# zhujinchong/3DGS-native

Measured on AMD Instinct MI355X. Metric: Mpixels/s forward+backward at 800x800, 1M Gaussians, higher is better.
Workload: dtype f32

## Files before the change

### 3dgs-native_amd/csrc/api.hip

```cpp
#include <stdio.h>
#include <stdlib.h>
#include <string.h>

#include <algorithm>
#include <atomic>
#include <mutex>
#include <vector>

#include "gsr_antialias.h"
#include "gsr_aux_grads.h"
#include "gsr_camera_grads.h"
#include "gsr_capacity.h"
#include "gsr_debug_layout.h"
#include "gsr_densify_stats.h"
#include "gsr_internal.h"

namespace {

#define HIP_TRY(expr)                                                                                                         \
    do {                                                                                                                      \
        hipError_t e_ = (expr);                                                                                               \
        if (e_ != hipSuccess) {                                                                                               \
            fprintf(stderr, "libgsr_hip: %s failed at %s:%d: %s\n", #expr, __FILE__, __LINE__, hipGetErrorString(e_));       \
            return GSR_E_HIP;                                                                                                 \
        }                                                                                                                     \
    } while (0)

struct Carver {
    char *p;
    size_t off = 0;
    explicit Carver(void *base) : p((char *)base) {}
    template <class T> T *take(size_t count)
    {
        T *r = (T *)(p ? p + off : nullptr);
        off += gsr_align(count * sizeof(T));
        return r;
    }
};

BinWs carve_bin(void *base, int64_t D)
{
    Carver c(base);
    BinWs w;
    w.hist = c.take<int32_t>(256 * ((size_t)gsr_radix_blocks(D) + 1));
    w.acc[0] = c.take<int32_t>(gsr_radix_acc_ints(D));
    w.acc[1] = c.take<int32_t>(gsr_radix_acc_ints(D));
    w.edge = c.take<int32_t>(3 * 256 * ((size_t)gsr_radix_blocks(D) + 1));
    w.tile_a = c.take<uint64_t>((size_t)D);
    w.tile_b = c.take<uint64_t>((size_t)D);
    w.bytes = c.off + 256;
    return w;
}

struct BwdWs {
    BlendRec *rec;
    GradRec *acc;
    size_t bytes;
};
BwdWs carve_bwd(void *base, int64_t N)
{
    Carver c(base);
    BwdWs w;
    w.rec = c.take<BlendRec>((size_t)N);
    w.acc = c.take<GradRec>((size_t)N);
    w.bytes = c.off + 256;
    return w;
}

int check_scene_cam(const GsrScene *sc, const GsrCamera *cam)
{
// ... 347 lines not shown
    HIP_TRY(hipMemsetAsync(image->inv_depth, 0, P * sizeof(float), s));
    HIP_TRY(hipMemsetAsync(image->final_T, 0, P * sizeof(float), s));
    HIP_TRY(hipMemsetAsync(image->n_contrib, 0, P * sizeof(int32_t), s));
    if (binning->backward_ws && N > 0) HIP_TRY(hipMemsetAsync(carve_bwd(binning->backward_ws, N).acc, 0, sizeof(GradRec) * (size_t)N, s));
    return GSR_OK;
}

int enqueue_render(const GsrScene *scene, const CamK &cam, const GsrGeom *geom, const GsrBinning *binning, const GsrImage *image,
                   const GeomWs &gw, const BinWs &bw, const int32_t *d_count, int64_t shape_D, hipStream_t s, int st)
{
    const int64_t N = scene->N, D = binning->D;
    const int tiles = cam.grid_x * cam.grid_y;
    if (!d_count) shape_D = D;
    mark(st, 4, s);
    const TilePlan plan = gsr_tile_plan(N, tiles);
    int32_t *order = binning->block_masks ? binning->block_order : nullptr;
    const bool file_order = order && tiles <= GSR_BO_MAX_TILES && gsr_bwd_block_px(N, shape_D, tiles) == 32;
    const bool use_fwd_order = fwd_order_wanted(tiles);
    HIP_TRY(gsr_launch_depth_block_offsets(gw, N, binning->ranges, 2 * tiles, bw.acc[0], (int)gsr_radix_acc_ints(D), order, order ? GSR_BO_HEADER : 0,
                                           file_order ? 1 : 0, s));
    mark(st, 5, s);
    HIP_TRY(gsr_launch_expand_blocks(plan, gw, bw, N, cam.grid_x, D, d_count, s));
    mark(st, 6, s);
    HIP_TRY(gsr_launch_tile_partition(plan, bw, binning->point_list, binning->ranges, D, d_count, s));
    mark(st, 7, s);
    mark(st, 8, s);
    void *clear = binning->backward_ws ? carve_bwd(binning->backward_ws, N).acc : nullptr;
    const size_t clear_bytes = clear ? sizeof(GradRec) * (size_t)N : 0;
    HIP_TRY(gsr_launch_blend_forward(cam, binning->ranges, binning->point_list, geom->blend_records ? (const BlendRec *)geom->blend_records : gw.rec, *image, binning->block_masks, file_order ? order : nullptr,
                                     clear, clear_bytes, s, use_fwd_order ? gw.fwd_order : nullptr, tiles <= GSR_FO_MAX_TILES ? gw.fwd_cost : nullptr,
                                     d_count, D));
    mark(st, 9, s);
    return GSR_OK;
}

}

extern "C" {

int gsr_forward_render(const GsrScene *scene, const GsrCamera *camera, const GsrGeom *geom, const GsrBinning *binning,
                       const GsrImage *image, void *geom_ws, size_t geom_ws_bytes, void *bin_ws, size_t bin_ws_bytes, void *stream)
{
    read_tuning();
    if (int rc = check_frame(scene, camera, binning, image)) return rc;
    const int64_t N = scene->N, D = binning->D;
    hipStream_t s = (hipStream_t)stream;
    const CamK cam = make_cam(camera);
// ... 314 lines not shown
```

### 3dgs-native_amd/csrc/gsr_internal.h

```cpp
#pragma once
#include <hip/hip_runtime.h>
#include <stdint.h>

#include "gsr.h"

#define GSR_WAVE 64

struct CamK {
    float view[16];
    float proj[16];
    float campos[3];
    float bg[3];
    float tan_fovx, tan_fovy;
    float focal_x, focal_y;
    int W, H, grid_x, grid_y;
};

struct __attribute__((aligned(16))) BlendRec {
    float f[16];
};

struct __attribute__((aligned(8))) TileRect {
    uint16_t x0, y0, x1, y1;
};
// ... 83 lines not shown
static inline int gsr_radix_sb(int nb)
{
    if (nb > GSR_RADIX_PREFIX_NB) return 32;
    int sb = 16;
    while ((int64_t)sb * sb < nb) ++sb;
    return sb;
}
static inline size_t gsr_radix_acc_ints(int64_t n)
{
    const int nb = (int)gsr_radix_blocks(n), sb = gsr_radix_sb(nb);
    return 256 * (size_t)(3 + nb / sb);
}
struct TilePlan {
    int tile_bits, id_bits;
    int item_bytes, id_shift;
    int npass;
    int bits[4];
    bool narrowing;
};
TilePlan gsr_tile_plan(int64_t N, int tiles);
struct BinWs {
    int32_t *hist;
    int32_t *acc[2];
    int32_t *edge;
    uint64_t *tile_a;
    uint64_t *tile_b;
    size_t bytes;
};
hipError_t gsr_launch_depth_block_offsets(const GeomWs &ws, int64_t n, int32_t *ranges, int ranges_n, int32_t *zero_acc, int zero_n, int32_t *zero_b,
                                          int zero_b_n, int bo_flag, hipStream_t s);
hipError_t gsr_launch_expand_blocks(const TilePlan &plan, const GeomWs &ws, const BinWs &bw, int64_t n, int grid_x, int64_t D, const int32_t *d_count,
                                    hipStream_t s);
hipError_t gsr_launch_tile_partition(const TilePlan &plan, const BinWs &bw, int32_t *point_list, int32_t *ranges, int64_t D, const int32_t *d_count,
                                     hipStream_t s);
#define GSR_BO_BANDS 8
#define GSR_BO_CLASSES 32
#define GSR_BO_SHARDS 16
#define GSR_BO_QUEUES (GSR_BO_BANDS * GSR_BO_CLASSES * GSR_BO_SHARDS)
#define GSR_BO_FLAG GSR_BO_QUEUES
#define GSR_BO_HEADER (GSR_BO_QUEUES + 4)
#define GSR_BO_MAX_TILES 4096
__host__ __device__ static inline int gsr_bo_tiles_per_band(int tiles) { return (tiles + GSR_BO_BANDS - 1) / GSR_BO_BANDS; }
__host__ __device__ static inline int gsr_bo_band(int tile, int tiles) { return tile / gsr_bo_tiles_per_band(tiles); }
static inline int gsr_bo_cap(int tiles) { return 8 * ((gsr_bo_tiles_per_band(tiles) + GSR_BO_SHARDS - 1) / GSR_BO_SHARDS); }
static inline size_t gsr_bo_ints(int tiles) { return GSR_BO_HEADER + (size_t)GSR_BO_QUEUES * (size_t)gsr_bo_cap(tiles); }
__host__ __device__ static inline int gsr_bo_class(int hits)
{
    if (hits < 8) return 0;
    const int lg = 31 - __builtin_clz((unsigned)hits);
    const int c = 1 + 4 * (lg - 3) + ((hits >> (lg - 2)) & 3);
    return c < GSR_BO_CLASSES ? c : GSR_BO_CLASSES - 1;
}
hipError_t gsr_launch_blend_forward(const CamK &cam, const int32_t *ranges, const int32_t *point_list,
                                    const BlendRec *rec, const GsrImage &img, uint8_t *block_masks ,
                                    int32_t *block_order ,
                                    void *clear, size_t clear_bytes , hipStream_t s,
                                    const int32_t *tile_order = nullptr , int32_t *tile_cost = nullptr ,
// ... 43 lines not shown
```

### 3dgs-native_amd/csrc/scan_sort.hip

```cpp
#include <algorithm>
#include <type_traits>
#include <utility>

#include "gsr_internal.h"

namespace {

__device__ __forceinline__ int wave_incl_scan(int v)
{
    asm("s_nop 1\n\tv_add_u32_dpp %0, %0, %0 row_shr:1 row_mask:0xf bank_mask:0xf\n\t"
        "s_nop 1\n\tv_add_u32_dpp %0, %0, %0 row_shr:2 row_mask:0xf bank_mask:0xf\n\t"
        "s_nop 1\n\tv_add_u32_dpp %0, %0, %0 row_shr:4 row_mask:0xf bank_mask:0xf\n\t"
        "s_nop 1\n\tv_add_u32_dpp %0, %0, %0 row_shr:8 row_mask:0xf bank_mask:0xf\n\t"
        "s_nop 1\n\tv_add_u32_dpp %0, %0, %0 row_bcast:15 row_mask:0xa bank_mask:0xf\n\t"
        "s_nop 1\n\tv_add_u32_dpp %0, %0, %0 row_bcast:31 row_mask:0xc bank_mask:0xf\n\t"
        "s_nop 1"
        : "+v"(v));
    return v;
}

__device__ __forceinline__ int block_incl_scan_256(int v, int *lds4 , int *total)
{
    const int lane = threadIdx.x & 63, w = threadIdx.x >> 6;
    int s = wave_incl_scan(v);
// ... 179 lines not shown
    int launched_first;
    int pack_ok;
};
__device__ __forceinline__ bool depth_items_packed(const DepthPass &dp, const DepthCtl &c) { return dp.pack_ok && c.npass >= 2 && c.npass <= 3; }
__device__ __forceinline__ unsigned long long depth_item_pack(uint32_t key, unsigned long long rect_raw, uint32_t id)
{
    const uint32_t r24 = (uint32_t)(rect_raw & 63ull) | ((uint32_t)((rect_raw >> 16) & 63ull) << 6) | ((uint32_t)((rect_raw >> 32) & 63ull) << 12) |
                         ((uint32_t)((rect_raw >> 48) & 63ull) << 18);
    return ((unsigned long long)((key >> 8) & 0xFFFFu) << 48) | ((unsigned long long)r24 << 24) | (unsigned long long)(id & 0xFFFFFFu);
}
__device__ __forceinline__ unsigned long long depth_item_rect(unsigned long long item)
{
    const uint32_t r24 = (uint32_t)(item >> 24) & 0xFFFFFFu;
    return (unsigned long long)(r24 & 63u) | ((unsigned long long)((r24 >> 6) & 63u) << 16) | ((unsigned long long)((r24 >> 12) & 63u) << 32) |
           ((unsigned long long)((r24 >> 18) & 63u) << 48);
}
template <bool DEPTH, int BITS, typename ItemT>
__device__ __forceinline__ int radix_digit(ItemT item, int shift, uint32_t kmin, uint32_t krange)
{
    if constexpr (DEPTH) return (int)((min((uint32_t)(item >> 32) - kmin, krange) >> shift) & 255u);
    else return (int)((item >> shift) & ((1 << BITS) - 1));
}

template <int RADIX_ITEMS, int BITS, typename ItemT, bool DEPTH>
__device__ __forceinline__ void radix_hist_block(const ItemT *__restrict__ in, int32_t *__restrict__ hist, int32_t *__restrict__ acc, int64_t n, int shift,
                                                 int sb, int block, uint32_t kmin, uint32_t krange, bool drop_culled)
{
    constexpr int CHUNK = 256 * RADIX_ITEMS;
    constexpr int RADIX = 1 << BITS;
    __shared__ int h[RADIX];
    if (threadIdx.x < RADIX) h[threadIdx.x] = 0;
    __syncthreads();
    const int64_t base = (int64_t)block * CHUNK;
    constexpr int VEC = 16 / (int)sizeof(ItemT);
    static_assert(RADIX_ITEMS % VEC == 0, "whole 16-byte loads per thread");
    struct alignas(16) Vec { ItemT v[VEC]; };
    Vec item[RADIX_ITEMS / VEC];
#pragma unroll
    for (int r = 0; r < RADIX_ITEMS / VEC; ++r) {
        const int64_t k = base + (int64_t)(r * 256 + (int)threadIdx.x) * VEC;
        if (k + VEC <= n) item[r] = *reinterpret_cast<const Vec *>(in + k);
        else {
#pragma unroll
            for (int j = 0; j < VEC; ++j) item[r].v[j] = k + j < n ? in[k + j] : (ItemT)0;
        }
    }
#pragma unroll
    for (int r = 0; r < RADIX_ITEMS / VEC; ++r) {
#pragma unroll
        for (int j = 0; j < VEC; ++j) {
            const int64_t k = base + (int64_t)(r * 256 + (int)threadIdx.x) * VEC + j;
            bool take = k < n;
            if constexpr (DEPTH) take = take && !(drop_culled && (uint32_t)(item[r].v[j] >> 32) == 0xFFFFFFFFu);
            if (take) atomicAdd(&h[radix_digit<DEPTH, BITS>(item[r].v[j], shift, kmin, krange)], 1);
        }
    }
    __syncthreads();
    if (threadIdx.x < RADIX) {
        const int c = h[threadIdx.x];
        hist[(size_t)block * RADIX + threadIdx.x] = c;
        if (c) atomicAdd(&acc[256 + (block / sb) * 256 + threadIdx.x], c);
    }
}

template <int RADIX_ITEMS, int BITS, typename ItemT, bool DEPTH = false>
__global__ __launch_bounds__(256) void radix_hist_kernel(const ItemT *__restrict__ in, int32_t *__restrict__ hist, int32_t *__restrict__ acc,
                                                         int64_t n, int shift, int sb, DepthPass dp)
{
    constexpr int CHUNK = 256 * RADIX_ITEMS;
    uint32_t kmin = 0u, krange = 0u;
    if constexpr (DEPTH) {
        const DepthCtl c = depth_ctl_load(dp.ctl, dp.force_npass);
        if (dp.pass < c.first || c.first < dp.launched_first) return;
        const int rel = dp.pass - c.first;
        if (rel == 0) return;
        in = reinterpret_cast<const ItemT *>(dp.buf[rel & 1]);
        shift = 8 * rel;
        kmin = c.min_bits; krange = c.range;
        if (depth_items_packed(dp, c)) { shift = 16 + 8 * (rel - 1); kmin = 0u; krange = 0xFFFFFFFFu; }
        n = c.n_vis;
        if ((int64_t)blockIdx.x * CHUNK >= n) return;
    }
    radix_hist_block<RADIX_ITEMS, BITS, ItemT, DEPTH>(in, hist, acc, n, shift, sb, (int)blockIdx.x, kmin, krange, false);
}
template <int RADIX_ITEMS, int BITS, typename ItemT>
__global__ __launch_bounds__(256) void radix_hist_cap_kernel(const ItemT *__restrict__ in, int32_t *__restrict__ hist, int32_t *__restrict__ acc,
                                                             int64_t n, int shift, int sb, const int32_t *__restrict__ d_count)
{
    radix_hist_block<RADIX_ITEMS, BITS, ItemT, false>(in, hist, acc, gsr_capped_count(d_count, n), shift, sb, (int)blockIdx.x, 0u, 0u, false);
}

template <int HIST_ITEMS>
__global__ __launch_bounds__(256) void scan_ctl_hist_kernel(const int32_t *__restrict__ in, const int32_t *__restrict__ wave_sums, int32_t *__restrict__ out,
                                                            int64_t n, int32_t *total_out, const uint32_t *__restrict__ blk_minmax, int nblk,
                                                            DepthCtlRaw *__restrict__ ctl, int n_ctl, int nb_scan,
                                                            const uint64_t *__restrict__ items, int32_t *__restrict__ hist, int32_t *__restrict__ acc_first, int sb)
{
    if ((int)blockIdx.x < nb_scan) {
        scan_final_block<0, 4>(in, wave_sums, out, n, total_out, (int)blockIdx.x);
    } else if ((int)blockIdx.x < nb_scan + n_ctl) {
        depth_ctl_from_blocks(blk_minmax, nblk, ctl, (int)blockIdx.x - nb_scan, n_ctl, total_out);
    } else {
        radix_hist_block<HIST_ITEMS, 8, uint64_t, true>(items, hist, acc_first, n, 0, sb, (int)blockIdx.x - nb_scan - n_ctl, 0u, 0xFFFFFFFFu, true);
    }
}

__global__ __launch_bounds__(1024) void radix_superscan_kernel(int32_t *__restrict__ acc, int nsuper, DepthPass dp)
{
    if (dp.ctl) {
        const DepthCtl c = depth_ctl_load(dp.ctl, dp.force_npass);
        if (dp.pass < c.first || c.first < dp.launched_first) return;
        if (dp.pass == c.first) acc = dp.acc_first;
    }
    __shared__ int4 s_part[64][16];
    const int ql = threadIdx.x & 15, g = threadIdx.x >> 4, q = (int)blockIdx.x * 16 + ql;
    const int per = (nsuper + 63) / 64, t0 = g * per, t1 = min(nsuper, t0 + per);
    int4 *rows = reinterpret_cast<int4 *>(acc + 256) + q;
    int4 sum = make_int4(0, 0, 0, 0);
    int4 v[8];
    const bool held = per <= 8;
    if (held) {
#pragma unroll
        for (int k = 0; k < 8; ++k) {
            v[k] = t0 + k < t1 ? rows[(size_t)(t0 + k) * 64] : make_int4(0, 0, 0, 0);
        }
#pragma unroll
// ... 22 lines not shown
            run.x += v[k].x; run.y += v[k].y; run.z += v[k].z; run.w += v[k].w;
        }
    } else {
        for (int tb = t0; tb < t1; tb += 8) {
#pragma unroll
            for (int k = 0; k < 8; ++k) v[k] = tb + k < t1 ? rows[(size_t)(tb + k) * 64] : make_int4(0, 0, 0, 0);
#pragma unroll
            for (int k = 0; k < 8; ++k) {
                if (tb + k < t1) rows[(size_t)(tb + k) * 64] = run;
                run.x += v[k].x; run.y += v[k].y; run.z += v[k].z; run.w += v[k].w;
            }
        }
    }
}

struct ScatterCarry {
    const TileRect *rect;
    TileRect *rect_sorted;
    int32_t *cnt_sorted;
    uint32_t *id_sorted;
    int64_t n_total;
};

struct ScatterFinal {
    int32_t *point_list;
    int32_t *ranges;
    int32_t *edge_first;
    int32_t *edge_last;
    int32_t *edge_pos;
    int32_t *totals;
    int id_shift;
    int narrow_id_bits;
    const int32_t *low_totals;
    int low_bits;
};

template <int RADIX_ITEMS, int BITS, typename ItemT, bool CARRY = false, bool FINAL = false, bool DEPTH = false, int THREADS = 256, bool LOWREC = false,
          bool PACKCAP = false, bool CAP = false>
__global__ __launch_bounds__(THREADS) void radix_scatter_kernel(const ItemT *__restrict__ in, ItemT *__restrict__ out,
                                                            const int32_t *__restrict__ hist, const int32_t *__restrict__ acc,
                                                            int64_t n, int shift, int nb, int sb, bool prefixed, int32_t *__restrict__ zero_acc,
                                                            int zero_n, ScatterCarry carry, ScatterFinal fin, DepthPass dp)
{
    constexpr int CHUNK = THREADS * RADIX_ITEMS;
    constexpr int NW = THREADS / 64;
    constexpr int RADIX = 1 << BITS;
    __shared__ ItemT s_items[CHUNK];
    __shared__ unsigned long long s_rect[(CARRY || PACKCAP) ? CHUNK : 1];
    __shared__ int s_wcnt[NW][RADIX];
    __shared__ int s_before[RADIX];
    __shared__ int s_total[RADIX];
    int *const s_dstart = s_total;
    int *const s_gbase = s_before;
    __shared__ int s_dcnt[FINAL ? RADIX : 1];
    __shared__ uint8_t s_low[LOWREC ? CHUNK : 1];
    __shared__ int s_seg[LOWREC ? 257 : 1];
    __shared__ int s_tmp[NW];
    __shared__ int s_valid_n;

    const int tid = threadIdx.x, lane = tid & 63, w = tid >> 6;
    const int64_t block_base = (int64_t)blockIdx.x * CHUNK;
    const int64_t wave_base = block_base + (int64_t)w * 64 * RADIX_ITEMS;
    const unsigned long long lt_mask = lane == 0 ? 0ull : (~0ull >> (64 - lane));

    if (tid < RADIX) {
#pragma unroll
        for (int k = 0; k < NW; ++k) s_wcnt[k][tid] = 0;
        s_before[tid] = 0;
        s_total[tid] = 0;
    }
    for (int z = blockIdx.x * THREADS + tid; z < zero_n; z += gridDim.x * THREADS) zero_acc[z] = 0;
    uint32_t kmin = 0u, krange = 0u;
    bool drop_culled = false;
    bool packed = false, pack_now = false, unpack = false;
    int64_t n_load = n;
    if constexpr (CAP) {
        n = n_load = gsr_capped_count(dp.count, n);
        if (block_base >= n) {
            if constexpr (FINAL)
                for (int d = tid; d < RADIX; d += THREADS) fin.edge_first[(size_t)d * nb + blockIdx.x] = -1;
            return;
        }
    }
    if constexpr (DEPTH) {
        const DepthCtl c = depth_ctl_load(dp.ctl, dp.force_npass);
        if (dp.pass < c.first || c.first < dp.launched_first) return;
        const int rel = dp.pass - c.first;
        if (rel == 0) acc = dp.acc_first;
        in = reinterpret_cast<const ItemT *>(dp.buf[rel & 1]);
        out = reinterpret_cast<ItemT *>(dp.buf[(rel + 1) & 1]);
        shift = 8 * rel;
        kmin = c.min_bits; krange = c.range;
        packed = depth_items_packed(dp, c);
        pack_now = PACKCAP && packed && rel == 0;
        if (packed && rel > 0) { shift = 16 + 8 * (rel - 1); kmin = 0u; krange = 0xFFFFFFFFu; unpack = true; }
        drop_culled = rel == 0;
        if (rel > 0) n = n_load = c.n_vis;
        if constexpr (CARRY) {
            const int64_t z0 = max((int64_t)c.n_vis, block_base), z1 = min(block_base + (int64_t)CHUNK, carry.n_total);
            for (int64_t z = z0 + tid; z < z1; z += THREADS) carry.cnt_sorted[z] = 0;
        }
        if (block_base >= n) return;
    }
    __syncthreads();
    if constexpr (LOWREC) {
        int tot;
        const int v = (tid < (1 << fin.low_bits)) ? fin.low_totals[tid] : 0;
        const int inc = block_incl_scan_nw<NW>(tid < 256 ? v : 0, s_tmp, &tot);
        if (tid < 256) s_seg[tid + 1] = inc;
        if (tid == 0) s_seg[0] = 0;
        __syncthreads();
    }

    int4 before_part = make_int4(0, 0, 0, 0), total_part = make_int4(0, 0, 0, 0);
    constexpr int TPT = RADIX / 4;
    {
        constexpr int GROUPS = THREADS / TPT;
        const int d4 = (tid % TPT) * 4, g = tid / TPT, my_sb = blockIdx.x / sb, nsuper = (nb + sb - 1) / sb;
        const int32_t *rows = hist + (size_t)my_sb * sb * RADIX + d4;
        const int within = (int)blockIdx.x - my_sb * sb;
#pragma unroll 4
        for (int t = g; t < within; t += GROUPS) {
            const int4 v = *reinterpret_cast<const int4 *>(rows + (size_t)t * RADIX);
            before_part.x += v.x; before_part.y += v.y; before_part.z += v.z; before_part.w += v.w;
        }
        if (prefixed) {
            if (g == 0) {
                total_part = *reinterpret_cast<const int4 *>(acc + d4);
                const int4 v = *reinterpret_cast<const int4 *>(acc + 256 + (size_t)my_sb * 256 + d4);
                before_part.x += v.x; before_part.y += v.y; before_part.z += v.z; before_part.w += v.w;
            }
        } else {
            const int32_t *sup = acc + 256 + d4;
#pragma unroll 4
            for (int t = g; t < nsuper; t += GROUPS) {
                const int4 v = *reinterpret_cast<const int4 *>(sup + (size_t)t * 256);
                total_part.x += v.x; total_part.y += v.y; total_part.z += v.z; total_part.w += v.w;
                if (t < my_sb) { before_part.x += v.x; before_part.y += v.y; before_part.z += v.z; before_part.w += v.w; }
            }
        }
    }
    {
        const int d4 = (tid % TPT) * 4;
        if (before_part.x) atomicAdd(&s_before[d4 + 0], before_part.x);
        if (before_part.y) atomicAdd(&s_before[d4 + 1], before_part.y);
        if (before_part.z) atomicAdd(&s_before[d4 + 2], before_part.z);
        if (before_part.w) atomicAdd(&s_before[d4 + 3], before_part.w);
        if (total_part.x) atomicAdd(&s_total[d4 + 0], total_part.x);
        if (total_part.y) atomicAdd(&s_total[d4 + 1], total_part.y);
        if (total_part.z) atomicAdd(&s_total[d4 + 2], total_part.z);
        if (total_part.w) atomicAdd(&s_total[d4 + 3], total_part.w);
    }

    ItemT item[RADIX_ITEMS];
    unsigned long long rc[(CARRY || PACKCAP) ? RADIX_ITEMS : 1];
    int rank[RADIX_ITEMS];
    uint8_t low[LOWREC ? RADIX_ITEMS : 1];
    bool valid_bits[RADIX_ITEMS];
#pragma unroll
    for (int r = 0; r < RADIX_ITEMS; ++r) {
        const int64_t k = wave_base + r * 64 + lane;
        const ItemT v = in[k < n_load ? k : n_load - 1];
        item[r] = k < n_load ? v : (ItemT)~(ItemT)0;
    }
    if constexpr (CARRY) {
        if (!unpack) {
#pragma unroll
            for (int r = 0; r < RADIX_ITEMS; ++r) {
                const int64_t k = wave_base + r * 64 + lane;
                const uint32_t id = k < n_load ? (uint32_t)item[r] : 0u;
                rc[r] = reinterpret_cast<const unsigned long long *>(carry.rect)[id];
            }
        } else {
#pragma unroll
            for (int r = 0; r < RADIX_ITEMS; ++r) rc[r] = depth_item_rect((unsigned long long)item[r]);
        }
    } else if constexpr (PACKCAP) {
        if (pack_now) {
#pragma unroll
            for (int r = 0; r < RADIX_ITEMS; ++r) {
                const int64_t k = wave_base + r * 64 + lane;
                rc[r] = reinterpret_cast<const unsigned long long *>(carry.rect)[k < n_load ? k : n_load - 1];
            }
        }
    }
#pragma unroll
    for (int r = 0; r < RADIX_ITEMS; ++r) {
        const int64_t k = wave_base + r * 64 + lane;
        bool valid = k < n;
        if constexpr (DEPTH) valid = valid && !(drop_culled && (uint32_t)(item[r] >> 32) == 0xFFFFFFFFu);
        valid_bits[r] = valid;
        if constexpr (LOWREC) {
            int p = 0;
#pragma unroll
            for (int step = 128; step >= 1; step >>= 1)
                if (s_seg[p + step] <= (int)min(k, n - 1)) p += step;
            low[r] = (uint8_t)p;
        }
        const int d = radix_digit<DEPTH, BITS>(item[r], shift, kmin, krange);
        unsigned int diff_lo = 0u, diff_hi = 0u;
#pragma unroll
        for (int b = 0; b < BITS; ++b) {
            const unsigned int rep = (unsigned int)__builtin_amdgcn_sbfe(d, b, 1);
            const unsigned long long m = __ballot(rep != 0u);
            diff_lo |= (unsigned int)m ^ rep;
            diff_hi |= (unsigned int)(m >> 32) ^ rep;
        }
        unsigned long long peers = ~(((unsigned long long)diff_hi << 32) | diff_lo) & __ballot(valid);
        if (!valid) peers = 0ull;
        const int before = __popcll(peers & lt_mask);
        const int old = valid ? s_wcnt[w][d] : 0;
        if (valid && before == 0) s_wcnt[w][d] = old + __popcll(peers);
        rank[r] = old + before;
    }
    __syncthreads();

    {
        const int d = tid;
        const bool own = d < RADIX;
        int run = 0;
        if (own) {
#pragma unroll
            for (int k = 0; k < NW; ++k) {
                const int c = s_wcnt[k][d];
                s_wcnt[k][d] = run;
                run += c;
            }
        }
        int tot;
        const int inc = block_incl_scan_nw<NW>(run, s_tmp, &tot);
        if (tid == 0) s_valid_n = tot;
        const int td = own ? s_total[d] : 0;
        const int before = own ? s_before[d] : 0;
        const int tinc = block_incl_scan_nw<NW>(td, s_tmp, &tot);
        if (own) {
            s_dstart[d] = inc - run;
            s_gbase[d] = tinc - td + before;
            if constexpr (!FINAL && sizeof(ItemT) == 8 && !DEPTH) {
                if (fin.totals && blockIdx.x == 0) fin.totals[d] = td;
            }
            if constexpr (FINAL) {
                if (blockIdx.x == 0) fin.totals[d] = td;
                s_dcnt[d] = run;
                if (run == 0) fin.edge_first[(size_t)d * nb + blockIdx.x] = -1;
            }
        }
    }
    __syncthreads();

#pragma unroll
    for (int r = 0; r < RADIX_ITEMS; ++r) {
        if (valid_bits[r]) {
            const int d = radix_digit<DEPTH, BITS>(item[r], shift, kmin, krange);
            const int slot = s_dstart[d] + s_wcnt[w][d] + rank[r];
            s_items[slot] = item[r];
            if constexpr (LOWREC) s_low[slot] = low[r];
            if constexpr (CARRY) s_rect[slot] = rc[r];
            else if constexpr (PACKCAP) { if (pack_now) s_rect[slot] = rc[r]; }
        }
    }
    __syncthreads();

    const int valid_n = s_valid_n;
#pragma unroll 4
    for (int r = 0; r < RADIX_ITEMS; ++r) {
        const int slot = r * THREADS + tid;
        if (slot < valid_n) {
            const ItemT it = s_items[slot];
            const int d = radix_digit<DEPTH, BITS>(it, shift, kmin, krange);
            const int64_t pos = (int64_t)s_gbase[d] + (slot - s_dstart[d]);
            if constexpr (FINAL) {
                uint32_t tile = (uint32_t)(it >> fin.id_shift);
                if constexpr (LOWREC) tile = (tile << fin.low_bits) | (uint32_t)s_low[slot];
                fin.point_list[pos] = (int32_t)(uint32_t)(it & (((ItemT)1 << fin.id_shift) - 1));
                const int rel = slot - s_dstart[d];
                const size_t e = (size_t)d * nb + blockIdx.x;
                if (rel > 0) {
                    uint32_t prev = (uint32_t)(s_items[slot - 1] >> fin.id_shift);
                    if constexpr (LOWREC) prev = (prev << fin.low_bits) | (uint32_t)s_low[slot - 1];
                    if (prev != tile) {
                        fin.ranges[2 * prev + 1] = (int32_t)pos;
                        fin.ranges[2 * tile] = (int32_t)pos;
                    }
                } else {
                    fin.edge_first[e] = (int32_t)tile;
                    fin.edge_pos[e] = (int32_t)pos;
                }
                if (rel == s_dcnt[d] - 1) fin.edge_last[e] = (int32_t)tile;
            } else if constexpr (CARRY) {
                carry.id_sorted[pos] = unpack ? ((uint32_t)it & 0xFFFFFFu) : (uint32_t)it;
            } else {
                bool narrowed = false;
                if constexpr (PACKCAP) {
                    if (pack_now) {
                        const uint32_t key = min((uint32_t)(it >> 32) - kmin, krange);
                        out[pos] = (ItemT)depth_item_pack(key, s_rect[slot], (uint32_t)it);
                        narrowed = true;
                    }
                }
                if constexpr (sizeof(ItemT) == 8 && !DEPTH) {
                    if (fin.narrow_id_bits) {
                        reinterpret_cast<uint32_t *>(out)[pos] = (uint32_t)(((it >> (shift + BITS)) << fin.narrow_id_bits) | (it & (((ItemT)1 << fin.narrow_id_bits) - 1)));
                        narrowed = true;
                    }
                }
                if (!narrowed) out[pos] = it;
            }
            if constexpr (CARRY) {
                const unsigned long long q = s_rect[slot];
                reinterpret_cast<unsigned long long *>(carry.rect_sorted)[pos] = q;
                const int x0 = (int)(q & 0xFFFF), y0 = (int)((q >> 16) & 0xFFFF), x1 = (int)((q >> 32) & 0xFFFF), y1 = (int)(q >> 48);
                carry.cnt_sorted[pos] = (x1 - x0) * (y1 - y0);
            }
        }
    }
}

__global__ __launch_bounds__(1024) void ranges_fixup_kernel(const int32_t *__restrict__ edge_first, const int32_t *__restrict__ edge_last,
                                                            const int32_t *__restrict__ edge_pos, const int32_t *__restrict__ totals, int nb,
                                                            int radix, int32_t *__restrict__ ranges)
{
    __shared__ int s_last[16];
    const int d = blockIdx.x, tid = threadIdx.x, lane = tid & 63, wv = tid >> 6;
    const int total = totals[d];
    if (total == 0) return;
    int digit_start = 0;
    for (int k = lane; k < d; k += 64) digit_start += totals[k];
#pragma unroll
    for (int o = 32; o >= 1; o >>= 1) digit_start += __shfl_xor(digit_start, o, 64);
    const size_t row = (size_t)d * nb;
    const int per = (nb + 15) / 16;
    const int b0 = wv * per, b1 = min(nb, b0 + per);
    int my_last = -1;
    for (int base = b0; base < b1; base += 64) {
        const int b = base + lane;
        const bool ne = b < b1 && edge_first[row + b] >= 0;
        const unsigned long long m = __ballot(ne);
        if (m) {
            const int hi = 63 - __builtin_clzll(m);
            my_last = __shfl(ne ? edge_last[row + b] : -1, hi, 64);
        }
    }
    if (lane == 0) s_last[wv] = my_last;
    __syncthreads();
    int carry = -1;
    for (int k = wv - 1; k >= 0; --k)
        if (s_last[k] >= 0) { carry = s_last[k]; break; }
    for (int base = b0; base < b1; base += 64) {
        const int b = base + lane;
        const bool ne = b < b1 && edge_first[row + b] >= 0;
        const int first = ne ? edge_first[row + b] : -1, last = ne ? edge_last[row + b] : -1, pos = ne ? edge_pos[row + b] : 0;
        const unsigned long long m = __ballot(ne);
        const unsigned long long below = m & (lane == 0 ? 0ull : (~0ull >> (64 - lane)));
        const int src = below ? 63 - __builtin_clzll(below) : 0;
        const int prev_in_chunk = __shfl(last, src, 64);
        const int prev = below ? prev_in_chunk : carry;
        if (ne) {
            if (prev < 0) ranges[2 * first] = pos;
            else if (prev != first) { ranges[2 * prev + 1] = pos; ranges[2 * first] = pos; }
        }
        if (m) carry = __shfl(last, 63 - __builtin_clzll(m), 64);
    }
    bool later = false;
    for (int k = wv + 1; k < 16; ++k) later = later || s_last[k] >= 0;
    if (!later && my_last >= 0 && lane == 0) ranges[2 * my_last + 1] = digit_start + total;
}

__global__ __launch_bounds__(1024) void depth_block_offsets_kernel(const int32_t *__restrict__ cnt_sorted, int64_t n, int32_t *__restrict__ pre256,
                                                                   int nsum, int32_t *__restrict__ sum4096, int32_t *__restrict__ ranges, int ranges_n,
                                                                   int32_t *__restrict__ zero_acc, int zero_n, int32_t *__restrict__ zero_b, int zero_b_n,
                                                                   int bo_flag)
{
    for (int64_t z = (int64_t)blockIdx.x * 1024 + threadIdx.x; z < zero_n; z += (int64_t)gridDim.x * 1024) zero_acc[z] = 0;
    for (int64_t z = (int64_t)blockIdx.x * 1024 + threadIdx.x; z < zero_b_n; z += (int64_t)gridDim.x * 1024) zero_b[z] = (z == GSR_BO_FLAG) ? bo_flag : 0;
    for (int64_t z = (int64_t)blockIdx.x * 1024 + threadIdx.x; z < ranges_n; z += (int64_t)gridDim.x * 1024) ranges[z] = 0;
    __shared__ int s_wsum[16];
    const int tid = threadIdx.x, lane = tid & 63, w = tid >> 6;
    const int blk = (int)blockIdx.x * 16 + w;
    int v = 0;
#pragma unroll
    for (int r = 0; r < 4; ++r) {
        const int64_t k = (int64_t)blk * 256 + r * 64 + lane;
        if (k < n) v += cnt_sorted[k];
    }
#pragma unroll
    for (int d = 32; d >= 1; d >>= 1) v += __shfl_xor(v, d, 64);
    if (lane == 0) s_wsum[w] = v;
    __syncthreads();
// ... 294 lines not shown
    return g;
}
template <int TIER> struct TierShape {
    static constexpr int CHUNK = TIER == 0 ? GSR_RADIX_TINY_CHUNK : TIER == 1 ? GSR_RADIX_SMALL_CHUNK : GSR_RADIX_CHUNK;
    static constexpr int WG = TIER == 0 ? 256 : TIER == 1 ? GSR_RADIX_SMALL_WG : GSR_RADIX_WG;
};
template <class F> static void with_tier(int tier, F &&f)
{
    if (tier == 0) f(std::integral_constant<int, 0>{});
    else if (tier == 1) f(std::integral_constant<int, 1>{});
    else f(std::integral_constant<int, 2>{});
}

template <int BITS, typename ItemT, bool CARRY, bool FINAL, bool DEPTH, bool LOWREC, bool PACKCAP>
static void radix_pass_launch(const ItemT *in, ItemT *out, int32_t *hist, int32_t *acc, int64_t n, int shift, int32_t *zero_acc, int zero_n,
                              const ScatterCarry &carry, const ScatterFinal &fin, const DepthPass &dp, bool hist_ready, const int32_t *d_count,
                              hipStream_t s)
{
    constexpr bool CAN_CAP = !CARRY && !DEPTH && !PACKCAP;
    const PassGeom g = pass_geom(n);
    with_tier(g.tier, [&](auto tier) {
        using T = TierShape<decltype(tier)::value>;
        constexpr int HIST_ITEMS = T::CHUNK / 256, ITEMS = T::CHUNK / T::WG;
        const dim3 grid(g.nb);
        if (hist_ready) {
        } else if (CAN_CAP && d_count) {
            if constexpr (CAN_CAP) hipLaunchKernelGGL((radix_hist_cap_kernel<HIST_ITEMS, BITS, ItemT>), grid, dim3(256), 0, s, in, hist, acc, n, shift, g.sb, d_count);
        } else {
            hipLaunchKernelGGL((radix_hist_kernel<HIST_ITEMS, BITS, ItemT, DEPTH>), grid, dim3(256), 0, s, in, hist, acc, n, shift, g.sb, dp);
        }
        if (g.prefixed) hipLaunchKernelGGL(radix_superscan_kernel, dim3(4), dim3(1024), 0, s, acc, (g.nb + g.sb - 1) / g.sb, dp);
        if (CAN_CAP && d_count) {
            DepthPass cdp{};
            cdp.count = d_count;
            if constexpr (CAN_CAP)
                hipLaunchKernelGGL((radix_scatter_kernel<ITEMS, BITS, ItemT, false, FINAL, false, T::WG, LOWREC, false, true>), grid, dim3(T::WG), 0, s, in, out,
                                   hist, acc, n, shift, g.nb, g.sb, g.prefixed, zero_acc, zero_n, carry, fin, cdp);
        } else {
            hipLaunchKernelGGL((radix_scatter_kernel<ITEMS, BITS, ItemT, CARRY, FINAL, DEPTH, T::WG, LOWREC, PACKCAP>), grid, dim3(T::WG), 0, s, in, out, hist,
                               acc, n, shift, g.nb, g.sb, g.prefixed, zero_acc, zero_n, carry, fin, dp);
        }
    });
    if constexpr (FINAL)
        hipLaunchKernelGGL(ranges_fixup_kernel, dim3(1 << BITS), dim3(1024), 0, s, fin.edge_first, fin.edge_last, fin.edge_pos, acc, g.nb, 1 << BITS,
                           fin.ranges);
}

template <bool FINAL>
static hipError_t tile_pass(int item_bytes, const void *in, void *out, int32_t *hist, int32_t *acc, int64_t n, int shift, int bits, int32_t *zero_acc,
                            const ScatterFinal &fin, const int32_t *d_count, hipStream_t s, bool hist_ready)
{
    const int zero_n = zero_acc ? (int)gsr_radix_acc_ints(n) : 0;
    auto launch = [&](auto item, auto digit) {
        using ItemT = decltype(item);
        constexpr int BITS = decltype(digit)::value;
        const ItemT *src = (const ItemT *)in;
        if constexpr (FINAL && sizeof(ItemT) == 4) {
            if (fin.low_bits) {
                radix_pass_launch<BITS, ItemT, false, true, false, true, false>(src, (ItemT *)out, hist, acc, n, shift, zero_acc, zero_n, ScatterCarry{}, fin,
                                                                                DepthPass{}, hist_ready, d_count, s);
                return;
            }
        }
        radix_pass_launch<BITS, ItemT, false, FINAL, false, false, false>(src, (ItemT *)out, hist, acc, n, shift, zero_acc, zero_n, ScatterCarry{}, fin,
                                                                          DepthPass{}, hist_ready, d_count, s);
    };
    auto with_bits = [&](auto item) {
        switch (bits) {
// ... 108 lines not shown
                       ranges_n, zero_acc, zero_n, zero_b, zero_b_n, bo_flag);
    return hipGetLastError();
}
hipError_t gsr_launch_expand_blocks(const TilePlan &plan, const GeomWs &ws, const BinWs &bw, int64_t n, int grid_x, int64_t D, const int32_t *d_count,
                                    hipStream_t s)
{
    if (n <= 0 || D <= 0) return hipSuccess;
    const PassGeom g = pass_geom(D);
    const int nsum = (int)gsr_div_up(n, 256), digit_mask = (1 << plan.bits[0]) - 1;
    auto launch = [&](auto *items) {
        using ItemT = std::remove_pointer_t<decltype(items)>;
        if (d_count)
            hipLaunchKernelGGL(expand_blocks_cap_kernel<ItemT>, dim3(g.nb), dim3(256), 0, s, ws.id_sorted, ws.cnt_sorted, ws.scan_tmp, ws.sum4096, nsum, ws.rect_sorted,
                               items, n, grid_x, D, plan.id_shift, g.chunk, digit_mask, bw.hist, bw.acc[0], g.sb, d_count);
        else
            hipLaunchKernelGGL(expand_blocks_kernel<ItemT>, dim3(g.nb), dim3(256), 0, s, ws.id_sorted, ws.cnt_sorted, ws.scan_tmp, ws.sum4096, nsum, ws.rect_sorted,
                               items, n, grid_x, D, plan.id_shift, g.chunk, digit_mask, bw.hist, bw.acc[0], g.sb);
    };
    if (plan.item_bytes == 4) launch((uint32_t *)bw.tile_a);
    else launch(bw.tile_a);
    return hipGetLastError();
}

hipError_t gsr_launch_tile_partition(const TilePlan &plan, const BinWs &bw, int32_t *point_list, int32_t *ranges, int64_t D, const int32_t *d_count,
                                     hipStream_t s)
{
    if (D <= 0) return hipSuccess;
    void *src = bw.tile_a, *dst = bw.tile_b;
    for (int pass = 0, shift = 0; pass < plan.npass; ++pass) {
        const int bits = plan.bits[pass];
        int32_t *acc = bw.acc[pass & 1], *next = bw.acc[(pass + 1) & 1];
        hipError_t e;
        if (pass + 1 < plan.npass) {
            ScatterFinal opt{};
            if (plan.narrowing) {
                opt.narrow_id_bits = plan.id_bits;
                opt.totals = acc;
            }
            e = tile_pass<false>(plan.item_bytes, src, dst, bw.hist, acc, D, plan.id_shift + shift, bits, next, opt, d_count, s, pass == 0);
        } else {
            const size_t per = ((size_t)1 << bits) * (size_t)gsr_radix_blocks(D);
            ScatterFinal fin{point_list, ranges, bw.edge, bw.edge + per, bw.edge + 2 * per, acc, plan.id_shift, 0, nullptr, 0};
            if (plan.narrowing) {
                fin.id_shift = plan.id_bits;
                fin.low_totals = next;
                fin.low_bits = plan.bits[0];
                e = tile_pass<true>(4, src, nullptr, bw.hist, acc, D, plan.id_bits, bits, nullptr, fin, d_count, s, false);
            } else {
                e = tile_pass<true>(plan.item_bytes, src, nullptr, bw.hist, acc, D, plan.id_shift + shift, bits, nullptr, fin, d_count, s, pass == 0);
            }
        }
        if (e != hipSuccess) return e;
        shift += bits;
        std::swap(src, dst);
    }
    return hipSuccess;
}
```

Baseline: 1181.

## Derive tile ranges from histogram counts instead of edge detection and fixup kernel

The final radix pass no longer tracks per-block edge tiles and then runs a separate ranges_fixup kernel. Per-tile counts are now accumulated during the histogram pass, using a small shared-memory window for the first tiles of each block and global atomics for the rest. An extra block in the scatter kernel then prefix-scans those counts into start/end ranges. This drops the edge workspace, one kernel launch and the per-element neighbour comparisons in the scatter, at the cost of more atomics in the histogram and a serial scan over all tiles in one block. It also adds launch-bounds occupancy hints to the final scatter.

```diff
diff --git a/3dgs-native_amd/csrc/api.hip b/3dgs-native_amd/csrc/api.hip
--- a/3dgs-native_amd/csrc/api.hip
+++ b/3dgs-native_amd/csrc/api.hip
@@ -45,7 +45,6 @@
     w.hist = c.take<int32_t>(256 * ((size_t)gsr_radix_blocks(D) + 1));
     w.acc[0] = c.take<int32_t>(gsr_radix_acc_ints(D));
     w.acc[1] = c.take<int32_t>(gsr_radix_acc_ints(D));
-    w.edge = c.take<int32_t>(3 * 256 * ((size_t)gsr_radix_blocks(D) + 1));
     w.tile_a = c.take<uint64_t>((size_t)D);
     w.tile_b = c.take<uint64_t>((size_t)D);
     w.bytes = c.off + 256;
@@ -439,7 +438,7 @@
     mark(st, 5, s);
     HIP_TRY(gsr_launch_expand_blocks(plan, gw, bw, N, cam.grid_x, D, d_count, s));
     mark(st, 6, s);
-    HIP_TRY(gsr_launch_tile_partition(plan, bw, binning->point_list, binning->ranges, D, d_count, s));
+    HIP_TRY(gsr_launch_tile_partition(plan, bw, binning->point_list, binning->ranges, tiles, D, d_count, s));
     mark(st, 7, s);
     mark(st, 8, s);
     void *clear = binning->backward_ws ? carve_bwd(binning->backward_ws, N).acc : nullptr;
diff --git a/3dgs-native_amd/csrc/gsr_internal.h b/3dgs-native_amd/csrc/gsr_internal.h
--- a/3dgs-native_amd/csrc/gsr_internal.h
+++ b/3dgs-native_amd/csrc/gsr_internal.h
@@ -129,7 +129,6 @@
 struct BinWs {
     int32_t *hist;
     int32_t *acc[2];
-    int32_t *edge;
     uint64_t *tile_a;
     uint64_t *tile_b;
     size_t bytes;
@@ -138,8 +137,8 @@
                                           int zero_b_n, int bo_flag, hipStream_t s);
 hipError_t gsr_launch_expand_blocks(const TilePlan &plan, const GeomWs &ws, const BinWs &bw, int64_t n, int grid_x, int64_t D, const int32_t *d_count,
                                     hipStream_t s);
-hipError_t gsr_launch_tile_partition(const TilePlan &plan, const BinWs &bw, int32_t *point_list, int32_t *ranges, int64_t D, const int32_t *d_count,
-                                     hipStream_t s);
+hipError_t gsr_launch_tile_partition(const TilePlan &plan, const BinWs &bw, int32_t *point_list, int32_t *ranges, int tiles, int64_t D,
+                                     const int32_t *d_count, hipStream_t s);
 #define GSR_BO_BANDS 8
 #define GSR_BO_CLASSES 32
 #define GSR_BO_SHARDS 16
diff --git a/3dgs-native_amd/csrc/scan_sort.hip b/3dgs-native_amd/csrc/scan_sort.hip
--- a/3dgs-native_amd/csrc/scan_sort.hip
+++ b/3dgs-native_amd/csrc/scan_sort.hip
@@ -225,14 +225,38 @@
     else return (int)((item >> shift) & ((1 << BITS) - 1));
 }
 
-template <int RADIX_ITEMS, int BITS, typename ItemT, bool DEPTH>
+struct ScatterFinal {
+    int32_t *point_list;
+    int32_t *ranges;
+    int tiles;
+    int count_is_digit;
+    int32_t *totals;
+    int id_shift;
+    int narrow_id_bits;
+    const int32_t *low_totals;
+    int low_bits;
+};
+
+constexpr int TILE_WIN = 2;
+template <int RADIX_ITEMS, int BITS, typename ItemT, bool DEPTH, bool TILES = false, bool LOWREC = false>
 __device__ __forceinline__ void radix_hist_block(const ItemT *__restrict__ in, int32_t *__restrict__ hist, int32_t *__restrict__ acc, int64_t n, int shift,
-                                                 int sb, int block, uint32_t kmin, uint32_t krange, bool drop_culled)
-{
+                                                 int sb, int block, uint32_t kmin, uint32_t krange, bool drop_culled, const ScatterFinal &fin)
+{
+    static_assert(!LOWREC || TILES, "the lower part is only wanted for the tile counts");
     constexpr int CHUNK = 256 * RADIX_ITEMS;
     constexpr int RADIX = 1 << BITS;
-    __shared__ int h[RADIX];
-    if (threadIdx.x < RADIX) h[threadIdx.x] = 0;
+    constexpr int ROWS = TILES ? TILE_WIN + 1 : 1;
+    __shared__ int h[ROWS * RADIX];
+    __shared__ int s_seg[LOWREC ? 257 : 1];
+    __shared__ int s_tmp[LOWREC ? 4 : 1];
+    for (int k = threadIdx.x; k < ROWS * RADIX; k += 256) h[k] = 0;
+    if constexpr (LOWREC) {
+        int tot;
+        const int v = ((int)threadIdx.x < (1 << fin.low_bits)) ? fin.low_totals[threadIdx.x] : 0;
+        const int inc = block_incl_scan_256(v, s_tmp, &tot);
+        s_seg[threadIdx.x + 1] = inc;
+        if (threadIdx.x == 0) s_seg[0] = 0;
+    }
     __syncthreads();
     const int64_t base = (int64_t)block * CHUNK;
     constexpr int VEC = 16 / (int)sizeof(ItemT);
@@ -248,6 +272,23 @@
             for (int j = 0; j < VEC; ++j) item[r].v[j] = k + j < n ? in[k + j] : (ItemT)0;
         }
     }
+    const int low_bits = !TILES ? 0 : LOWREC ? fin.low_bits : shift - fin.id_shift;
+    const uint32_t low_mask = (1u << low_bits) - 1u;
+    auto low_of = [&](ItemT it, int64_t k) -> uint32_t {
+        if constexpr (LOWREC) {
+            int p = 0;
+#pragma unroll
+            for (int step = 128; step >= 1; step >>= 1)
+                if (s_seg[p + step] <= (int)k) p += step;
+            return (uint32_t)p;
+        } else {
+            return (uint32_t)(it >> fin.id_shift) & low_mask;
+        }
+    };
+    uint32_t low0 = 0u;
+    if constexpr (TILES) {
+        if (base < n) low0 = low_of(in[base], base);
+    }
 #pragma unroll
     for (int r = 0; r < RADIX_ITEMS / VEC; ++r) {
 #pragma unroll
@@ -255,20 +296,42 @@
             const int64_t k = base + (int64_t)(r * 256 + (int)threadIdx.x) * VEC + j;
             bool take = k < n;
             if constexpr (DEPTH) take = take && !(drop_culled && (uint32_t)(item[r].v[j] >> 32) == 0xFFFFFFFFu);
-            if (take) atomicAdd(&h[radix_digit<DEPTH, BITS>(item[r].v[j], shift, kmin, krange)], 1);
-        }
-    }
-    __syncthreads();
+            if (take) {
+                const int d = radix_digit<DEPTH, BITS>(item[r].v[j], shift, kmin, krange);
+                if constexpr (TILES) {
+                    const uint32_t low = low_of(item[r].v[j], k), row = low - low0;
+                    if (row < (uint32_t)TILE_WIN) atomicAdd(&h[(int)row * RADIX + d], 1);
+                    else {
+                        atomicAdd(&h[TILE_WIN * RADIX + d], 1);
+                        const uint32_t tile = ((uint32_t)d << low_bits) | low;
+                        if (tile < (uint32_t)fin.tiles) atomicAdd(&fin.ranges[2 * (size_t)tile + 1], 1);
+                    }
+                } else {
+                    atomicAdd(&h[d], 1);
+                }
+            }
+        }
+    }
+    __syncthreads();
+    if constexpr (TILES) {
+        for (int k = threadIdx.x; k < TILE_WIN * RADIX; k += 256) {
+            const int c = h[k];
+            const uint32_t tile = ((uint32_t)(k & (RADIX - 1)) << low_bits) | (low0 + (uint32_t)(k >> BITS));
+            if (c && tile < (uint32_t)fin.tiles) atomicAdd(&fin.ranges[2 * (size_t)tile + 1], c);
+        }
+    }
     if (threadIdx.x < RADIX) {
-        const int c = h[threadIdx.x];
+        int c = 0;
+#pragma unroll
+        for (int row = 0; row < ROWS; ++row) c += h[row * RADIX + threadIdx.x];
         hist[(size_t)block * RADIX + threadIdx.x] = c;
         if (c) atomicAdd(&acc[256 + (block / sb) * 256 + threadIdx.x], c);
     }
 }
 
-template <int RADIX_ITEMS, int BITS, typename ItemT, bool DEPTH = false>
+template <int RADIX_ITEMS, int BITS, typename ItemT, bool DEPTH = false, bool TILES = false, bool LOWREC = false>
 __global__ __launch_bounds__(256) void radix_hist_kernel(const ItemT *__restrict__ in, int32_t *__restrict__ hist, int32_t *__restrict__ acc,
-                                                         int64_t n, int shift, int sb, DepthPass dp)
+                                                         int64_t n, int shift, int sb, DepthPass dp, ScatterFinal fin)
 {
     constexpr int CHUNK = 256 * RADIX_ITEMS;
     uint32_t kmin = 0u, krange = 0u;
@@ -284,13 +347,14 @@
         n = c.n_vis;
         if ((int64_t)blockIdx.x * CHUNK >= n) return;
     }
-    radix_hist_block<RADIX_ITEMS, BITS, ItemT, DEPTH>(in, hist, acc, n, shift, sb, (int)blockIdx.x, kmin, krange, false);
-}
-template <int RADIX_ITEMS, int BITS, typename ItemT>
+    radix_hist_block<RADIX_ITEMS, BITS, ItemT, DEPTH, TILES, LOWREC>(in, hist, acc, n, shift, sb, (int)blockIdx.x, kmin, krange, false, fin);
+}
+template <int RADIX_ITEMS, int BITS, typename ItemT, bool TILES, bool LOWREC>
 __global__ __launch_bounds__(256) void radix_hist_cap_kernel(const ItemT *__restrict__ in, int32_t *__restrict__ hist, int32_t *__restrict__ acc,
-                                                             int64_t n, int shift, int sb, const int32_t *__restrict__ d_count)
-{
-    radix_hist_block<RADIX_ITEMS, BITS, ItemT, false>(in, hist, acc, gsr_capped_count(d_count, n), shift, sb, (int)blockIdx.x, 0u, 0u, false);
+                                                             int64_t n, int shift, int sb, const int32_t *__restrict__ d_count, ScatterFinal fin)
+{
+    radix_hist_block<RADIX_ITEMS, BITS, ItemT, false, TILES, LOWREC>(in, hist, acc, gsr_capped_count(d_count, n), shift, sb, (int)blockIdx.x, 0u, 0u, false,
+                                                                     fin);
 }
 
 template <int HIST_ITEMS>
@@ -304,7 +368,7 @@
     } else if ((int)blockIdx.x < nb_scan + n_ctl) {
         depth_ctl_from_blocks(blk_minmax, nblk, ctl, (int)blockIdx.x - nb_scan, n_ctl, total_out);
     } else {
-        radix_hist_block<HIST_ITEMS, 8, uint64_t, true>(items, hist, acc_first, n, 0, sb, (int)blockIdx.x - nb_scan - n_ctl, 0u, 0xFFFFFFFFu, true);
+        radix_hist_block<HIST_ITEMS, 8, uint64_t, true>(items, hist, acc_first, n, 0, sb, (int)blockIdx.x - nb_scan - n_ctl, 0u, 0xFFFFFFFFu, true, ScatterFinal{});
     }
 }
 
@@ -373,22 +437,55 @@
     int64_t n_total;
 };
 
-struct ScatterFinal {
-    int32_t *point_list;
-    int32_t *ranges;
-    int32_t *edge_first;
-    int32_t *edge_last;
-    int32_t *edge_pos;
-    int32_t *totals;
-    int id_shift;
-    int narrow_id_bits;
-    const int32_t *low_totals;
-    int low_bits;
-};
-
-template <int RADIX_ITEMS, int BITS, typename ItemT, bool CARRY = false, bool FINAL = false, bool DEPTH = false, int THREADS = 256, bool LOWREC = false,
-          bool PACKCAP = false, bool CAP = false>
-__global__ __launch_bounds__(THREADS) void radix_scatter_kernel(const ItemT *__restrict__ in, ItemT *__restrict__ out,
+template <int THREADS, int RADIX>
+__device__ __forceinline__ void ranges_from_counts(const ScatterFinal &fin, const int32_t *__restrict__ acc, int nb, int sb, bool prefixed, int *s_cnt ,
+                                                   int *s_tmp )
+{
+    constexpr int NW = THREADS / 64, PER = 4096 / THREADS;
+    const int tid = threadIdx.x;
+    if (fin.count_is_digit) {
+        if (tid < RADIX) {
+            int c = 0;
+            if (prefixed) c = acc[tid];
+            else {
+#pragma unroll 4
+                for (int t = 0, nsuper = (nb + sb - 1) / sb; t < nsuper; ++t) c += acc[256 + (size_t)t * 256 + tid];
+            }
+            s_cnt[tid] = c;
+        }
+        __syncthreads();
+    }
+    int2 *const r2 = reinterpret_cast<int2 *>(fin.ranges);
+    int carry = 0;
+#pragma unroll 1
+    for (int t0 = 0; t0 < fin.tiles; t0 += 4096) {
+        const int tb = t0 + tid * PER;
+        int c[PER], sum = 0;
+#pragma unroll
+        for (int j = 0; j < PER; ++j) {
+            const int t = tb + j;
+            c[j] = t >= fin.tiles ? 0 : !fin.count_is_digit ? fin.ranges[2 * (size_t)t + 1] : t < RADIX ? s_cnt[t] : 0;
+        }
+#pragma unroll
+        for (int j = 0; j < PER; ++j) sum += c[j];
+        int tot;
+        int run = carry + block_incl_scan_nw<NW>(sum, s_tmp, &tot) - sum;
+#pragma unroll
+        for (int j = 0; j < PER; ++j) {
+            if (c[j] > 0) r2[tb + j] = make_int2(run, run + c[j]);
+            run += c[j];
+        }
+        carry += tot;
+    }
+}
+
+constexpr int scatter_min_waves(bool final_pass, size_t item_bytes, int chunk, int bits)
+{
+    return !final_pass ? 1 : !(item_bytes == 8 && chunk == 4096 && bits >= 7) ? 8 : bits == 7 ? 7 : 6;
+}
+template <int RADIX_ITEMS, int BITS, typename ItemT, bool CARRY = false, bool FINAL = false, bool DEPTH = false, int THREADS = 256, bool PACKCAP = false,
+          bool CAP = false>
+__global__ __launch_bounds__(THREADS, scatter_min_waves(FINAL, sizeof(ItemT), THREADS * RADIX_ITEMS, BITS)) void radix_scatter_kernel(const ItemT *__restrict__ in, ItemT *__restrict__ out,
                                                             const int32_t *__restrict__ hist, const int32_t *__restrict__ acc,
                                                             int64_t n, int shift, int nb, int sb, bool prefixed, int32_t *__restrict__ zero_acc,
                                                             int zero_n, ScatterCarry carry, ScatterFinal fin, DepthPass dp)
@@ -403,13 +500,16 @@
     __shared__ int s_total[RADIX];
     int *const s_dstart = s_total;
     int *const s_gbase = s_before;
-    __shared__ int s_dcnt[FINAL ? RADIX : 1];
-    __shared__ uint8_t s_low[LOWREC ? CHUNK : 1];
-    __shared__ int s_seg[LOWREC ? 257 : 1];
     __shared__ int s_tmp[NW];
     __shared__ int s_valid_n;
 
     const int tid = threadIdx.x, lane = tid & 63, w = tid >> 6;
+    if constexpr (FINAL) {
+        if ((int)blockIdx.x == nb) {
+            ranges_from_counts<THREADS, RADIX>(fin, acc, nb, sb, prefixed, s_total, s_tmp);
+            return;
+        }
+    }
     const int64_t block_base = (int64_t)blockIdx.x * CHUNK;
     const int64_t wave_base = block_base + (int64_t)w * 64 * RADIX_ITEMS;
     const unsigned long long lt_mask = lane == 0 ? 0ull : (~0ull >> (64 - lane));
@@ -427,11 +527,7 @@
     int64_t n_load = n;
     if constexpr (CAP) {
         n = n_load = gsr_capped_count(dp.count, n);
-        if (block_base >= n) {
-            if constexpr (FINAL)
-                for (int d = tid; d < RADIX; d += THREADS) fin.edge_first[(size_t)d * nb + blockIdx.x] = -1;
-            return;
-        }
+        if (block_base >= n) return;
     }
     if constexpr (DEPTH) {
         const DepthCtl c = depth_ctl_load(dp.ctl, dp.force_npass);
@@ -454,14 +550,6 @@
         if (block_base >= n) return;
     }
     __syncthreads();
-    if constexpr (LOWREC) {
-        int tot;
-        const int v = (tid < (1 << fin.low_bits)) ? fin.low_totals[tid] : 0;
-        const int inc = block_incl_scan_nw<NW>(tid < 256 ? v : 0, s_tmp, &tot);
-        if (tid < 256) s_seg[tid + 1] = inc;
-        if (tid == 0) s_seg[0] = 0;
-        __syncthreads();
-    }
 
     int4 before_part = make_int4(0, 0, 0, 0), total_part = make_int4(0, 0, 0, 0);
     constexpr int TPT = RADIX / 4;
@@ -506,7 +594,6 @@
     ItemT item[RADIX_ITEMS];
     unsigned long long rc[(CARRY || PACKCAP) ? RADIX_ITEMS : 1];
     int rank[RADIX_ITEMS];
-    uint8_t low[LOWREC ? RADIX_ITEMS : 1];
     bool valid_bits[RADIX_ITEMS];
 #pragma unroll
     for (int r = 0; r < RADIX_ITEMS; ++r) {
@@ -541,13 +628,6 @@
         bool valid = k < n;
         if constexpr (DEPTH) valid = valid && !(drop_culled && (uint32_t)(item[r] >> 32) == 0xFFFFFFFFu);
         valid_bits[r] = valid;
-        if constexpr (LOWREC) {
-            int p = 0;
-#pragma unroll
-            for (int step = 128; step >= 1; step >>= 1)
-                if (s_seg[p + step] <= (int)min(k, n - 1)) p += step;
-            low[r] = (uint8_t)p;
-        }
         const int d = radix_digit<DEPTH, BITS>(item[r], shift, kmin, krange);
         unsigned int diff_lo = 0u, diff_hi = 0u;
 #pragma unroll
@@ -590,11 +670,6 @@
             if constexpr (!FINAL && sizeof(ItemT) == 8 && !DEPTH) {
                 if (fin.totals && blockIdx.x == 0) fin.totals[d] = td;
             }
-            if constexpr (FINAL) {
-                if (blockIdx.x == 0) fin.totals[d] = td;
-                s_dcnt[d] = run;
-                if (run == 0) fin.edge_first[(size_t)d * nb + blockIdx.x] = -1;
-            }
         }
     }
     __syncthreads();
@@ -605,7 +680,6 @@
             const int d = radix_digit<DEPTH, BITS>(item[r], shift, kmin, krange);
             const int slot = s_dstart[d] + s_wcnt[w][d] + rank[r];
             s_items[slot] = item[r];
-            if constexpr (LOWREC) s_low[slot] = low[r];
             if constexpr (CARRY) s_rect[slot] = rc[r];
             else if constexpr (PACKCAP) { if (pack_now) s_rect[slot] = rc[r]; }
         }
@@ -621,23 +695,7 @@
             const int d = radix_digit<DEPTH, BITS>(it, shift, kmin, krange);
             const int64_t pos = (int64_t)s_gbase[d] + (slot - s_dstart[d]);
             if constexpr (FINAL) {
-                uint32_t tile = (uint32_t)(it >> fin.id_shift);
-                if constexpr (LOWREC) tile = (tile << fin.low_bits) | (uint32_t)s_low[slot];
                 fin.point_list[pos] = (int32_t)(uint32_t)(it & (((ItemT)1 << fin.id_shift) - 1));
-                const int rel = slot - s_dstart[d];
-                const size_t e = (size_t)d * nb + blockIdx.x;
-                if (rel > 0) {
-                    uint32_t prev = (uint32_t)(s_items[slot - 1] >> fin.id_shift);
-                    if constexpr (LOWREC) prev = (prev << fin.low_bits) | (uint32_t)s_low[slot - 1];
-                    if (prev != tile) {
-                        fin.ranges[2 * prev + 1] = (int32_t)pos;
-                        fin.ranges[2 * tile] = (int32_t)pos;
-                    }
-                } else {
-                    fin.edge_first[e] = (int32_t)tile;
-                    fin.edge_pos[e] = (int32_t)pos;
-                }
-                if (rel == s_dcnt[d] - 1) fin.edge_last[e] = (int32_t)tile;
             } else if constexpr (CARRY) {
                 carry.id_sorted[pos] = unpack ? ((uint32_t)it & 0xFFFFFFu) : (uint32_t)it;
             } else {
@@ -665,56 +723,6 @@
             }
         }
     }
-}
-
-__global__ __launch_bounds__(1024) void ranges_fixup_kernel(const int32_t *__restrict__ edge_first, const int32_t *__restrict__ edge_last,
-                                                            const int32_t *__restrict__ edge_pos, const int32_t *__restrict__ totals, int nb,
-                                                            int radix, int32_t *__restrict__ ranges)
-{
-    __shared__ int s_last[16];
-    const int d = blockIdx.x, tid = threadIdx.x, lane = tid & 63, wv = tid >> 6;
-    const int total = totals[d];
-    if (total == 0) return;
-    int digit_start = 0;
-    for (int k = lane; k < d; k += 64) digit_start += totals[k];
-#pragma unroll
-    for (int o = 32; o >= 1; o >>= 1) digit_start += __shfl_xor(digit_start, o, 64);
-    const size_t row = (size_t)d * nb;
-    const int per = (nb + 15) / 16;
-    const int b0 = wv * per, b1 = min(nb, b0 + per);
-    int my_last = -1;
-    for (int base = b0; base < b1; base += 64) {
-        const int b = base + lane;
-        const bool ne = b < b1 && edge_first[row + b] >= 0;
-        const unsigned long long m = __ballot(ne);
-        if (m) {
-            const int hi = 63 - __builtin_clzll(m);
-            my_last = __shfl(ne ? edge_last[row + b] : -1, hi, 64);
-        }
-    }
-    if (lane == 0) s_last[wv] = my_last;
-    __syncthreads();
-    int carry = -1;
-    for (int k = wv - 1; k >= 0; --k)
-        if (s_last[k] >= 0) { carry = s_last[k]; break; }
-    for (int base = b0; base < b1; base += 64) {
-        const int b = base + lane;
-        const bool ne = b < b1 && edge_first[row + b] >= 0;
-        const int first = ne ? edge_first[row + b] : -1, last = ne ? edge_last[row + b] : -1, pos = ne ? edge_pos[row + b] : 0;
-        const unsigned long long m = __ballot(ne);
-        const unsigned long long below = m & (lane == 0 ? 0ull : (~0ull >> (64 - lane)));
-        const int src = below ? 63 - __builtin_clzll(below) : 0;
-        const int prev_in_chunk = __shfl(last, src, 64);
-        const int prev = below ? prev_in_chunk : carry;
-        if (ne) {
-            if (prev < 0) ranges[2 * first] = pos;
-            else if (prev != first) { ranges[2 * prev + 1] = pos; ranges[2 * first] = pos; }
-        }
-        if (m) carry = __shfl(last, 63 - __builtin_clzll(m), 64);
-    }
-    bool later = false;
-    for (int k = wv + 1; k < 16; ++k) later = later || s_last[k] >= 0;
-    if (!later && my_last >= 0 && lane == 0) ranges[2 * my_last + 1] = digit_start + total;
 }
 
 __global__ __launch_bounds__(1024) void depth_block_offsets_kernel(const int32_t *__restrict__ cnt_sorted, int64_t n, int32_t *__restrict__ pre256,
@@ -1055,28 +1063,26 @@
     with_tier(g.tier, [&](auto tier) {
         using T = TierShape<decltype(tier)::value>;
         constexpr int HIST_ITEMS = T::CHUNK / 256, ITEMS = T::CHUNK / T::WG;
-        const dim3 grid(g.nb);
+        const dim3 grid(g.nb), scatter_grid(g.nb + (FINAL ? 1 : 0));
         if (hist_ready) {
         } else if (CAN_CAP && d_count) {
-            if constexpr (CAN_CAP) hipLaunchKernelGGL((radix_hist_cap_kernel<HIST_ITEMS, BITS, ItemT>), grid, dim3(256), 0, s, in, hist, acc, n, shift, g.sb, d_count);
+            if constexpr (CAN_CAP)
+                hipLaunchKernelGGL((radix_hist_cap_kernel<HIST_ITEMS, BITS, ItemT, FINAL, LOWREC>), grid, dim3(256), 0, s, in, hist, acc, n, shift, g.sb, d_count, fin);
         } else {
-            hipLaunchKernelGGL((radix_hist_kernel<HIST_ITEMS, BITS, ItemT, DEPTH>), grid, dim3(256), 0, s, in, hist, acc, n, shift, g.sb, dp);
+            hipLaunchKernelGGL((radix_hist_kernel<HIST_ITEMS, BITS, ItemT, DEPTH, FINAL, LOWREC>), grid, dim3(256), 0, s, in, hist, acc, n, shift, g.sb, dp, fin);
         }
         if (g.prefixed) hipLaunchKernelGGL(radix_superscan_kernel, dim3(4), dim3(1024), 0, s, acc, (g.nb + g.sb - 1) / g.sb, dp);
         if (CAN_CAP && d_count) {
             DepthPass cdp{};
             cdp.count = d_count;
             if constexpr (CAN_CAP)
-                hipLaunchKernelGGL((radix_scatter_kernel<ITEMS, BITS, ItemT, false, FINAL, false, T::WG, LOWREC, false, true>), grid, dim3(T::WG), 0, s, in, out,
+                hipLaunchKernelGGL((radix_scatter_kernel<ITEMS, BITS, ItemT, false, FINAL, false, T::WG, false, true>), scatter_grid, dim3(T::WG), 0, s, in, out,
                                    hist, acc, n, shift, g.nb, g.sb, g.prefixed, zero_acc, zero_n, carry, fin, cdp);
         } else {
-            hipLaunchKernelGGL((radix_scatter_kernel<ITEMS, BITS, ItemT, CARRY, FINAL, DEPTH, T::WG, LOWREC, PACKCAP>), grid, dim3(T::WG), 0, s, in, out, hist,
+            hipLaunchKernelGGL((radix_scatter_kernel<ITEMS, BITS, ItemT, CARRY, FINAL, DEPTH, T::WG, PACKCAP>), scatter_grid, dim3(T::WG), 0, s, in, out, hist,
                                acc, n, shift, g.nb, g.sb, g.prefixed, zero_acc, zero_n, carry, fin, dp);
         }
     });
-    if constexpr (FINAL)
-        hipLaunchKernelGGL(ranges_fixup_kernel, dim3(1 << BITS), dim3(1024), 0, s, fin.edge_first, fin.edge_last, fin.edge_pos, acc, g.nb, 1 << BITS,
-                           fin.ranges);
 }
 
 template <bool FINAL>
@@ -1231,8 +1237,8 @@
     return hipGetLastError();
 }
 
-hipError_t gsr_launch_tile_partition(const TilePlan &plan, const BinWs &bw, int32_t *point_list, int32_t *ranges, int64_t D, const int32_t *d_count,
-                                     hipStream_t s)
+hipError_t gsr_launch_tile_partition(const TilePlan &plan, const BinWs &bw, int32_t *point_list, int32_t *ranges, int tiles, int64_t D,
+                                     const int32_t *d_count, hipStream_t s)
 {
     if (D <= 0) return hipSuccess;
     void *src = bw.tile_a, *dst = bw.tile_b;
@@ -1248,8 +1254,7 @@
             }
             e = tile_pass<false>(plan.item_bytes, src, dst, bw.hist, acc, D, plan.id_shift + shift, bits, next, opt, d_count, s, pass == 0);
         } else {
-            const size_t per = ((size_t)1 << bits) * (size_t)gsr_radix_blocks(D);
-            ScatterFinal fin{point_list, ranges, bw.edge, bw.edge + per, bw.edge + 2 * per, acc, plan.id_shift, 0, nullptr, 0};
+            ScatterFinal fin{point_list, ranges, tiles, plan.npass == 1, nullptr, plan.id_shift, 0, nullptr, 0};
             if (plan.narrowing) {
                 fin.id_shift = plan.id_bits;
                 fin.low_totals = next;
```

Result: no change. 1196 (median of 6 runs) (+1.3%).
